# zachramsey/pm-rl

Hardware: AMD Instinct MI355X
Metric: env-steps/sec (whole node) at 65k envs x 30 assets; reward MAE vs CPU ref (higher is better)
Workload: dtype f64

## Files before the change

pm-rl_amd/csrc/step_relay.h:

```cpp
#pragma once
#include "env_step.h"
#include "scalar_vec.h"

namespace pmenv_dev {

struct RelayParams {
    uint32_t scal;
    uint32_t epoch;
    uint64_t* w;
    uint64_t* list;
    uint32_t* done;
    uint32_t spin;
    uint32_t rot;
    uint32_t grid;
    const int32_t* kp_in;
    int32_t* kp_out;
    const float* halo_in;
    float* halo_out;
    uint32_t* seq;
    int32_t* kp;
    float* halo;
    uint32_t B;
    uint32_t halo_stride;
    const float* obs;
    uint32_t par;
};
enum { kSeqD = 0, kSeqE = 1, kSeqV = 2, kSeqC = 3, kSeqEC = 4, kSeqHobs = 6 };

struct RelayCtx {
    uint32_t epoch;
    const int32_t* kp_in;
    int32_t* kp_out;
    const float* halo_in;
    float* halo_out;
};
template <bool SEQ>
__device__ __forceinline__ RelayCtx relay_ctx(const RelayParams& r) {
    RelayCtx c{r.epoch, r.kp_in, r.kp_out, r.halo_in, r.halo_out};
    if constexpr (SEQ) {
        const uint32_t par = __builtin_amdgcn_readfirstlane(r.seq[kSeqC]);
        c.epoch = __builtin_amdgcn_readfirstlane(r.seq[kSeqEC]);
        c.kp_in = r.kp + (size_t)par * r.B;
        c.kp_out = r.kp + (size_t)(par ^ 1u) * r.B;
        c.halo_in = r.halo + (size_t)par * r.halo_stride;
        c.halo_out = r.halo + (size_t)(par ^ 1u) * r.halo_stride;
    }
    return c;
}

struct KArgs {
    StepParams p;
    RelayParams r;
    uint32_t qtot;
};
__device__ __forceinline__ KArgs kargs() {
    typedef __attribute__((address_space(4))) const uint32_t KWord;
    KWord* ka = (KWord*)__builtin_amdgcn_kernarg_segment_ptr();
    asm volatile("" : "+s"(ka));
    uint32_t w[sizeof(KArgs) / 4];
#pragma unroll
    for (size_t i = 0; i < sizeof(KArgs) / 4; ++i) w[i] = ka[i];
    KArgs k;
    __builtin_memcpy(&k, w, sizeof(KArgs));
    return k;
}

constexpr uint32_t kStampSlots = 16, kStampMaxWg = 40960;
static __device__ uint64_t* g_relay_stamps;
template <bool ST, bool DRAIN = false>
__device__ __forceinline__ uint64_t relay_clock(uint32_t dep) {
    uint64_t t = 0;
    if constexpr (ST) {
        if constexpr (DRAIN)
            asm volatile("s_waitcnt vmcnt(0)\n\ts_memrealtime %0\n\ts_waitcnt lgkmcnt(0)" : "=s"(t) : "v"(dep) : "memory");
        else
            asm volatile("s_memrealtime %0\n\ts_waitcnt lgkmcnt(0)" : "=s"(t) : "v"(dep) : "memory");
    }
    return t;
}
template <bool ST, int K>
__device__ __forceinline__ void relay_stamps_put(uint32_t bid, uint32_t epoch, const uint64_t (&ts)[K]) {
    if constexpr (ST) {
        uint64_t* s = g_relay_stamps;
        if (s && threadIdx.x == 0 && bid < kStampMaxWg) {
#pragma unroll
            for (int k = 0; k < K; ++k) s[((size_t)(epoch % kStampSlots) * kStampMaxWg + bid) * 8 + k] = ts[k];
        }
    }
}

__device__ __forceinline__ void relay_put(uint64_t* w, uint32_t epoch, uint32_t bits) {
    __hip_atomic_store(w, ((uint64_t)epoch << 32) | bits, __ATOMIC_RELAXED, __HIP_MEMORY_SCOPE_AGENT);
}
__device__ __forceinline__ uint64_t relay_get(const uint64_t* w) {
    return __hip_atomic_load(const_cast<uint64_t*>(w), __ATOMIC_RELAXED, __HIP_MEMORY_SCOPE_AGENT);
}

__device__ __forceinline__ uint32_t relay_list_read(const RelayParams& r, uint32_t epoch) {
    __atomic_signal_fence(__ATOMIC_SEQ_CST);
    __builtin_amdgcn_s_waitcnt(0);
    __atomic_signal_fence(__ATOMIC_SEQ_CST);
    const uint64_t lw = relay_get(r.list);
    return (uint32_t)(lw >> 32) == epoch ? (uint32_t)lw : 0u;
}

template <int BLOCK, int KL, int KA, bool ST = false>
__device__ __forceinline__ uint32_t relay_scalar(const StepParams& p, const RelayParams& r, int s, uint32_t epoch,
                                                 int32_t* kp_out, uint64_t t_entry = 0) {
    uint64_t ts[3] = {t_entry, 0, 0};
    constexpr int EPW = 64 / KL, EPB = (BLOCK / 64) * EPW;
    const int lane = threadIdx.x & 63;
    const int b = s * EPB + (int)(threadIdx.x >> 6) * EPW + lane / KL;
    const int j = lane % KL;
    const int N = p.N;
    const bool env_ok = b < p.B;
    uint32_t listed;
    if constexpr (KA == 0) {
        const ScalarIn in = scalar_load<KL>(p, b, lane);
        const ScalarMid m = scalar_core<KL>(p, b, lane, in);
        if (env_ok && j < N) relay_put(r.w + (size_t)b * N + j, epoch, __float_as_uint(m.wp));
        if (env_ok && j == 0) kp_out[b] = m.k + 1;
        listed = relay_list_read(r, epoch);
        ts[1] = relay_clock<ST>(listed);
        scalar_tail<KL>(p, b, lane, in, m);
    } else {
        const VecIn<KA> in = vec_load<KL, KA, true>(p, b, lane);
        const VecMid<KA> m = vec_core<KL, KA, true>(p, b, lane, in);
#pragma unroll
        for (int e = 0; e < KA; ++e) {
            const int n = j + e * KL;
            if (env_ok && n < N) relay_put(r.w + (size_t)b * N + n, epoch, __float_as_uint(m.wp[e]));
        }
        if (env_ok && j == 0) kp_out[b] = in.k + 1;
        listed = relay_list_read(r, epoch);
        ts[1] = relay_clock<ST>(listed);
        vec_tail<KL, KA, true>(p, b, lane, in, m);
    }
    ts[2] = relay_clock<ST, true>(0);
    relay_stamps_put<ST>((uint32_t)s, epoch, ts);
    return listed;
}

template <int BLOCK, int V, int POL, bool OUT, bool ADOPT, bool ST = false>
__device__ __forceinline__ bool relay_tile(const StepParams& p, const RelayParams& r, uint32_t qtot, uint32_t spin, uint32_t t,
                                           uint32_t epoch, const int32_t* kp_in, const float* halo_in,
                                           float* halo_out, f4* sh4, f4* sh_bar, float* sh_wp, int32_t* sh_kc,
                                           int32_t* sh_ok, uint64_t t_entry = 0) {
    uint64_t ts[6] = {t_entry, 0, 0, 0, 0, 0};
    constexpr int kAux = POL == 1 ? 2 : 0;
    constexpr int CPW = BLOCK * V, F = 5;
    const int tid = threadIdx.x, lane = tid & 63, wave = tid >> 6;
    const uint32_t c0 = t * CPW;
    const uint32_t nblk = min((uint32_t)CPW, qtot - c0);
    const auto rs = make_rsrc(p.obs + (size_t)c0 * 4, nblk * 16u);
    f4 own[V];
#pragma unroll
    for (int v = 0; v < V; ++v) own[v] = buf_load4<kAux>(rs, (uint32_t)(64 * V * wave + 64 * v + lane) * 16u);
    const uint32_t ntiles = (qtot + CPW - 1) / CPW;
    const uint32_t nh = t + 1 < ntiles ? min(2u, qtot - c0 - nblk) : 0u;
    const float* hsrc = OUT ? p.obs + (size_t)(c0 + nblk) * 4 : halo_in + (size_t)t * 8;
    const f4 hal = buf_load4<0>(make_rsrc(hsrc, nh * 16u), tid < 2 ? (uint32_t)tid * 16u : 0xFFFFFFF0u);
    __builtin_amdgcn_sched_barrier(0);
    const int N = p.N, W = p.W, WF = W * F;
    const uint32_t per4 = (uint32_t)(N * WF) >> 2;
    const uint32_t b_lo = fdiv(c0, p.div_units);
    const uint32_t g_lo = b_lo * (uint32_t)N + fdiv(4u * (c0 - b_lo * per4), p.div_wf);
    const uint32_t ql = c0 + nblk - 1u;
    const uint32_t b_hi = fdiv(ql, p.div_units);
    const uint32_t g_hi = b_hi * (uint32_t)N + fdiv(4u * (ql - b_hi * per4) + 3u, p.div_wf);
    const bool mine = (uint32_t)tid <= g_hi - g_lo;
    const uint32_t g = g_lo + (mine ? (uint32_t)tid : 0u);
    const uint32_t b = g / (uint32_t)N, n = g - b * (uint32_t)N;
    const float* barb = env_bar(p, (int)b);
    const float nanv = __int_as_float(0x7fc00000);
    f4 xb = f4{nanv, nanv, nanv, nanv};
    int32_t kc = 0;
    uint64_t ww = 0;
    if (barb) xb = *reinterpret_cast<const f4*>(barb + (size_t)n * 4);
    kc = kp_in[b];
    ww = relay_get(r.w + g);
    bool ready = !mine || (uint32_t)(ww >> 32) == epoch;
    ts[1] = relay_clock<ST>((uint32_t)ww);
    for (uint32_t polls = 0; !ADOPT && !__all(ready) && polls < spin; ++polls) {
        __builtin_amdgcn_s_sleep(2);
        if (!ready) {
            ww = relay_get(r.w + g);
            ready = (uint32_t)(ww >> 32) == epoch;
        }
    }
    const bool wave_ok = __all(ready);
    ts[2] = relay_clock<ST>((uint32_t)ww);
    if (mine) {
        sh_bar[tid] = xb;
        sh_wp[tid] = __uint_as_float((uint32_t)ww);
        sh_kc[tid] = kc;
    }
#pragma unroll
    for (int v = 0; v < V; ++v) sh4[64 * V * wave + 64 * v + lane] = own[v];
    if (tid < 2) sh4[CPW + tid] = hal;
    if (lane == 0) sh_ok[wave] = wave_ok ? 1 : 0;
    __syncthreads();
    ts[3] = relay_clock<ST>(0);
    if constexpr (ADOPT) {
        bool tile_ok = true;
#pragma unroll
        for (int w = 0; w < BLOCK / 64; ++w) tile_ok = tile_ok && sh_ok[w] != 0;
        if (!tile_ok) return false;
        if (tid == 0)
            sh_ok[BLOCK / 64] = __hip_atomic_exchange(r.done + t, epoch, __ATOMIC_RELAXED, __HIP_MEMORY_SCOPE_AGENT) != epoch;
        __syncthreads();
        if (!sh_ok[BLOCK / 64]) return true;
    }
    const auto rd = OUT ? make_rsrc(p.obs_out + (size_t)c0 * 4, nblk * 16u) : rs;
    const bool first_out = !OUT && t > 0;
    bool ok = true;
#pragma unroll
    for (int v = 0; v < V; ++v) {
        const int j = 64 * V * wave + 64 * v + lane;
        const uint32_t q = min(c0 + (uint32_t)j, qtot - 1u);
        const uint32_t bq = fdiv(q, p.div_units);
        const uint32_t j0 = 4u * (q - bq * per4);
        const uint32_t row = fdiv(j0, p.div_wf);
        const int kk = (int)(j0 - row * (uint32_t)WF);
        const int i = (int)(bq * (uint32_t)N + row - g_lo);
        const f4 n1 = sh4[j + 1], n2 = sh4[j + 2];
        const float sh[4] = {n1.y, n1.z, n1.w, n2.x};
        const float un[4] = {own[v].x, own[v].y, own[v].z, own[v].w};
        f4 o = compose2(p, kk, sh_kc[i], un, sh, [&](f4& x, float& xwp) {
            x = sh_bar[i];
            xwp = sh_wp[i];
        });
        if (!ADOPT && v == 0) {
            int32_t okv = 1;
#pragma unroll
            for (int w = 0; w < BLOCK / 64; ++w) okv &= sh_ok[w];
            ok = __builtin_amdgcn_readfirstlane(okv) != 0;
        }
        buf_store4<kAux>(rd, ok ? (uint32_t)j * 16u : 0x80000000u, o);
        if (ok && first_out && j < 2) reinterpret_cast<f4*>(halo_out)[2 * (t - 1) + j] = o;
    }
    ts[4] = relay_clock<ST>(0);
    ts[5] = relay_clock<ST, true>(0);
    relay_stamps_put<ST>(r.scal + t, epoch, ts);
    return ok;
}

template <int BLOCK, int V, int POL, bool OUT, bool SEQ>
__device__ __forceinline__ void relay_adopt(f4* sh4, f4* sh_bar, float* sh_wp, int32_t* sh_kc, int32_t* sh_ok,
                                            uint32_t listed) {
    constexpr int kB = BLOCK / 64 + 1;
    const int wave = threadIdx.x >> 6;
    if ((threadIdx.x & 63) == 0) sh_ok[wave] = (int32_t)__builtin_amdgcn_readfirstlane(listed);
    __syncthreads();
    uint32_t n = 0;
#pragma unroll
    for (int w = 0; w < BLOCK / 64; ++w) n = max(n, (uint32_t)sh_ok[w]);
    if (n == 0) return;
    const KArgs ka = kargs();
    const RelayCtx c = relay_ctx<SEQ>(ka.r);
    for (uint32_t i = 0; i < n; ++i) {
        __syncthreads();
        if (threadIdx.x == 0) {
            const uint64_t e = relay_get(ka.r.list + 1 + i);
            int32_t t = (uint32_t)(e >> 32) == c.epoch ? (int32_t)(uint32_t)e : -1;
            if (t >= 0 && __hip_atomic_load(ka.r.done + t, __ATOMIC_RELAXED, __HIP_MEMORY_SCOPE_AGENT) == c.epoch)
                t = -1;
            sh_ok[kB] = t;
        }
        __syncthreads();
        const int32_t t = __builtin_amdgcn_readfirstlane(sh_ok[kB]);
        if (t >= 0)
            (void)relay_tile<BLOCK, V, POL, OUT, true>(ka.p, ka.r, ka.qtot, 0u, (uint32_t)t, c.epoch, c.kp_in, c.halo_in,
                                                       c.halo_out, sh4, sh_bar, sh_wp, sh_kc, sh_ok);
    }
}

template <int BLOCK, int V, int POL, bool OUT, bool SEQ>
__device__ __forceinline__ void relay_defer(uint32_t t, f4* sh4, f4* sh_bar, float* sh_wp, int32_t* sh_kc,
                                            int32_t* sh_ok) {
    const KArgs ka = kargs();
    const RelayCtx c = relay_ctx<SEQ>(ka.r);
    if (threadIdx.x == 0) {
        uint64_t lw = relay_get(ka.r.list), nw;
        do {
            nw = (uint32_t)(lw >> 32) == c.epoch ? lw + 1 : ((uint64_t)c.epoch << 32) | 1u;
        } while (!__hip_atomic_compare_exchange_strong(ka.r.list, &lw, nw, __ATOMIC_RELAXED, __ATOMIC_RELAXED,
                                                        __HIP_MEMORY_SCOPE_AGENT));
        const uint32_t slot = (uint32_t)(lw >> 32) == c.epoch ? (uint32_t)lw : 0u;
        relay_put(ka.r.list + 1 + slot, c.epoch, t);
        __atomic_signal_fence(__ATOMIC_SEQ_CST);
        __builtin_amdgcn_s_waitcnt(0);
        __atomic_signal_fence(__ATOMIC_SEQ_CST);
    }
    __syncthreads();
    (void)relay_tile<BLOCK, V, POL, OUT, true>(ka.p, ka.r, ka.qtot, 0u, t, c.epoch, c.kp_in, c.halo_in, c.halo_out, sh4,
                                               sh_bar, sh_wp, sh_kc, sh_ok);
}

template <int BLOCK, int V, int POL, bool OUT, int KL, int KA, int OCC = 1, bool SEQ = false, int ANY = 0>
__global__ __launch_bounds__(BLOCK) __attribute__((amdgpu_waves_per_eu(OCC))) void step_relay_kernel(
    StepParams p, RelayParams r, uint32_t qtot) {
    __shared__ f4 sh4[BLOCK * V + 2];
    __shared__ f4 sh_bar[BLOCK];
    __shared__ float sh_wp[BLOCK];
    __shared__ int32_t sh_kc[BLOCK];
    __shared__ int32_t sh_ok[BLOCK / 64 + 2];
    const RelayCtx c = relay_ctx<SEQ>(r);
    if constexpr (SEQ) {
        if (blockIdx.x == 0 && threadIdx.x == 0) {
            const uint64_t hobs = OUT ? 0ull : (uint64_t)(uintptr_t)r.obs;
            r.seq[kSeqD] = (uint32_t)((c.kp_in - r.kp) / r.B) ^ 1u;
            r.seq[kSeqE] = c.epoch;
            r.seq[kSeqV] = 1u;
            r.seq[kSeqHobs] = (uint32_t)hobs;
            r.seq[kSeqHobs + 1] = (uint32_t)(hobs >> 32);
        }
    }
    constexpr bool kSt = ANY == 2;
    const uint64_t t_entry = relay_clock<kSt>(0);
    uint32_t bid = blockIdx.x;
    if constexpr (ANY == 1) {
        bid += r.rot;
        if (bid >= r.grid) bid -= r.grid;
    }
    if (bid < r.scal) {
        const uint32_t listed = relay_scalar<BLOCK, KL, KA, kSt>(p, r, (int)bid, c.epoch, c.kp_out, t_entry);
        relay_adopt<BLOCK, V, POL, OUT, SEQ>(sh4, sh_bar, sh_wp, sh_kc, sh_ok, listed);
    } else if (!relay_tile<BLOCK, V, POL, OUT, false, kSt>(p, r, qtot, ANY == 1 ? r.spin : kRelaySpin, bid - r.scal, c.epoch,
                                                           c.kp_in, c.halo_in, c.halo_out, sh4, sh_bar, sh_wp, sh_kc,
                                                           sh_ok, t_entry)) {
        relay_defer<BLOCK, V, POL, OUT, SEQ>(bid - r.scal, sh4, sh_bar, sh_wp, sh_kc, sh_ok);
    }
}

static __global__ __launch_bounds__(256) void relay_prime_kernel(StepParams p, RelayParams r, int prime_kp, int seq) {
    uint32_t d = r.par;
    bool kp = prime_kp != 0, halo = p.halo != nullptr;
    if (seq) {
        d = __builtin_amdgcn_readfirstlane(r.seq[kSeqD]);
        const uint32_t e = __builtin_amdgcn_readfirstlane(r.seq[kSeqE]);
        const uint32_t v = __builtin_amdgcn_readfirstlane(r.seq[kSeqV]);
        const uint64_t hobs = (uint64_t)__builtin_amdgcn_readfirstlane(r.seq[kSeqHobs]) |
                              ((uint64_t)__builtin_amdgcn_readfirstlane(r.seq[kSeqHobs + 1]) << 32);
        kp = v == 0;
        halo = halo && (v == 0 || hobs != (uint64_t)(uintptr_t)p.obs);
        if (blockIdx.x == 0 && threadIdx.x == 0) {
            r.seq[kSeqC] = d;
            r.seq[kSeqEC] = e + 1u == 0u ? 1u : e + 1u;
        }
    }
    if (halo) {
        p.halo += (size_t)d * r.halo_stride;
        copy_halo(p);
    }
    if (kp) {
        int32_t* kpd = r.kp + (size_t)d * r.B;
        for (int b = blockIdx.x * blockDim.x + threadIdx.x; b < p.B; b += gridDim.x * blockDim.x) kpd[b] = p.k[b];
    }
}

}
```

Baseline: 105.0 million.

## Add uniform-shift fast path that scatters new row cells into LDS image

Adds a fast path to the non-adopt relay tile. When every row in the block agrees on whether the weight slot shifts, each row owner writes its new bar values and weight straight into the shared tile image. Every output vector is then just a four-float shifted read, with an optional keep-weight select, instead of the per-element compose2 with its fdiv index math and per-row lookups. The cost is an extra __syncthreads, more registers for the per-row cell offsets, and overwriting sh4, so the fallback path now reads own values back from shared memory.

```diff
diff --git a/pm-rl_amd/csrc/compose_cells.h b/pm-rl_amd/csrc/compose_cells.h
--- /dev/null
+++ b/pm-rl_amd/csrc/compose_cells.h
@@ -0,0 +1,57 @@
+#pragma once
+
+#include <stdint.h>
+
+#if defined(__HIPCC__)
+#define PMENV_CELLS_HD __host__ __device__ inline
+#else
+#define PMENV_CELLS_HD inline
+#endif
+
+namespace compose_cells {
+
+constexpr int kF = 5;
+constexpr int kCells = 5;
+constexpr int kNoWeight = 4;
+
+PMENV_CELLS_HD bool shape_ok(int64_t N, int64_t W) { return N >= 1 && W >= 2 && (N * W * kF) % 4 == 0; }
+
+PMENV_CELLS_HD bool shift_w(bool ring_storage, int32_t k, int W) { return !(ring_storage && k >= W - 1); }
+
+PMENV_CELLS_HD int32_t slot_pos(int32_t k, int W) { return (int32_t)(((uint32_t)k + 1u) % (uint32_t)W) * kF + (kF - 1); }
+
+struct RowCells {
+    int32_t off[kCells];
+    uint32_t in;
+    bool shift_w;
+};
+
+PMENV_CELLS_HD RowCells row_cells_rel(int W, int32_t img, int32_t rel, int32_t k, bool ring_storage) {
+    RowCells c;
+    const int32_t WF = W * kF;
+    c.shift_w = shift_w(ring_storage, k, W);
+    for (int f = 0; f < kF - 1; ++f) c.off[f] = rel + WF + f;
+    c.off[kF - 1] = c.shift_w ? rel + WF + (kF - 1) : rel + slot_pos(k, W);
+    c.in = 0;
+    for (int i = 0; i < kCells; ++i) c.in |= (uint32_t)(c.off[i] >= 0 && c.off[i] < img) << i;
+    return c;
+}
+
+PMENV_CELLS_HD RowCells row_cells(int64_t N, int W, uint64_t c0, int32_t img, uint64_t g, int32_t k, bool ring_storage) {
+    (void)N;
+    const int64_t WF = (int64_t)W * kF;
+    const int64_t rel = (int64_t)g * WF - 4 * (int64_t)c0;
+    if (rel <= -WF - kCells || rel >= (int64_t)img) {
+        RowCells c;
+        for (int i = 0; i < kCells; ++i) c.off[i] = -1;
+        c.in = 0;
+        c.shift_w = shift_w(ring_storage, k, W);
+        return c;
+    }
+    return row_cells_rel(W, img, (int32_t)rel, k, ring_storage);
+}
+
+PMENV_CELLS_HD int weight_elem(uint64_t q) { return (int)((q + 4u) % 5u); }
+PMENV_CELLS_HD int weight_elem_tile(uint32_t c0_mod5, uint32_t j) { return (int)((c0_mod5 + j + 4u) % 5u); }
+
+}
diff --git a/pm-rl_amd/csrc/step_relay.h b/pm-rl_amd/csrc/step_relay.h
--- a/pm-rl_amd/csrc/step_relay.h
+++ b/pm-rl_amd/csrc/step_relay.h
@@ -1,4 +1,7 @@
 #pragma once
+#include <type_traits>
+
+#include "compose_cells.h"
 #include "env_step.h"
 #include "scalar_vec.h"
 
@@ -164,7 +167,9 @@
     const int N = p.N, W = p.W, WF = W * F;
     const uint32_t per4 = (uint32_t)(N * WF) >> 2;
     const uint32_t b_lo = fdiv(c0, p.div_units);
-    const uint32_t g_lo = b_lo * (uint32_t)N + fdiv(4u * (c0 - b_lo * per4), p.div_wf);
+    const uint32_t f_lo = 4u * (c0 - b_lo * per4);
+    const uint32_t r_lo = fdiv(f_lo, p.div_wf);
+    const uint32_t g_lo = b_lo * (uint32_t)N + r_lo;
     const uint32_t ql = c0 + nblk - 1u;
     const uint32_t b_hi = fdiv(ql, p.div_units);
     const uint32_t g_hi = b_hi * (uint32_t)N + fdiv(4u * (ql - b_hi * per4) + 3u, p.div_wf);
@@ -189,6 +194,16 @@
         }
     }
     const bool wave_ok = __all(ready);
+    const bool ring_st = p.ring_mode == PMENV_RING_STORAGE;
+    const bool row_sh = compose_cells::shift_w(ring_st, kc, W);
+    int32_t vote = wave_ok ? 1 : 0;
+    compose_cells::RowCells rc{};
+    if constexpr (!ADOPT) {
+        vote |= (__all(!mine || row_sh) ? 2 : 0) | (__all(!mine || !row_sh) ? 4 : 0);
+        const int32_t rel = (int32_t)(r_lo * (uint32_t)WF) - (int32_t)f_lo + tid * WF;
+        rc = compose_cells::row_cells_rel(W, 4 * (CPW + 2), rel, kc, ring_st);
+        if (!mine) rc.in = 0;
+    }
     ts[2] = relay_clock<ST>((uint32_t)ww);
     if (mine) {
         sh_bar[tid] = xb;
@@ -198,7 +213,7 @@
 #pragma unroll
     for (int v = 0; v < V; ++v) sh4[64 * V * wave + 64 * v + lane] = own[v];
     if (tid < 2) sh4[CPW + tid] = hal;
-    if (lane == 0) sh_ok[wave] = wave_ok ? 1 : 0;
+    if (lane == 0) sh_ok[wave] = vote;
     __syncthreads();
     ts[3] = relay_clock<ST>(0);
     if constexpr (ADOPT) {
@@ -214,6 +229,49 @@
     const auto rd = OUT ? make_rsrc(p.obs_out + (size_t)c0 * 4, nblk * 16u) : rs;
     const bool first_out = !OUT && t > 0;
     bool ok = true;
+    if constexpr (!ADOPT) {
+        int32_t okv = 7;
+#pragma unroll
+        for (int w = 0; w < BLOCK / 64; ++w) okv &= sh_ok[w];
+        okv = __builtin_amdgcn_readfirstlane(okv);
+        ok = (okv & 1) != 0;
+        if (okv & 6) {
+            if (rc.in) {
+                float* img = reinterpret_cast<float*>(sh4);
+                const float pv[compose_cells::kCells] = {xb.x, xb.y, xb.z, xb.w, __uint_as_float((uint32_t)ww)};
+#pragma unroll
+                for (int i = 0; i < compose_cells::kCells; ++i)
+                    if (rc.in >> i & 1u) img[rc.off[i]] = pv[i];
+            }
+            __syncthreads();
+            const uint32_t c0m = c0 % 5u;
+            const uint32_t soff = ok ? 0u : 0x80000000u;
+            auto shift_all = [&](auto keep_w) {
+#pragma unroll
+                for (int v = 0; v < V; ++v) {
+                    const int j = 64 * V * wave + 64 * v + lane;
+                    const f4 n1 = sh4[j + 1], n2 = sh4[j + 2];
+                    f4 o = f4{n1.y, n1.z, n1.w, n2.x};
+                    if constexpr (decltype(keep_w)::value) {
+                        const f4 n0 = sh4[j];
+                        const int ew = compose_cells::weight_elem_tile(c0m, (uint32_t)j);
+                        o.x = pick(ew == 0, n0.x, o.x);
+                        o.y = pick(ew == 1, n0.y, o.y);
+                        o.z = pick(ew == 2, n0.z, o.z);
+                        o.w = pick(ew == 3, n0.w, o.w);
+                    }
+                    buf_store4<kAux>(rd, soff + (uint32_t)j * 16u, o);
+                    if (v == 0 && ok && first_out && j < 2) reinterpret_cast<f4*>(halo_out)[2 * (t - 1) + j] = o;
+                }
+            };
+            if (okv & 4) shift_all(std::true_type{});
+            else shift_all(std::false_type{});
+            ts[4] = relay_clock<ST>(0);
+            ts[5] = relay_clock<ST, true>(0);
+            relay_stamps_put<ST>(r.scal + t, epoch, ts);
+            return ok;
+        }
+    }
 #pragma unroll
     for (int v = 0; v < V; ++v) {
         const int j = 64 * V * wave + 64 * v + lane;
@@ -223,19 +281,14 @@
         const uint32_t row = fdiv(j0, p.div_wf);
         const int kk = (int)(j0 - row * (uint32_t)WF);
         const int i = (int)(bq * (uint32_t)N + row - g_lo);
+        const f4 n0 = ADOPT ? own[v] : sh4[j];
         const f4 n1 = sh4[j + 1], n2 = sh4[j + 2];
         const float sh[4] = {n1.y, n1.z, n1.w, n2.x};
-        const float un[4] = {own[v].x, own[v].y, own[v].z, own[v].w};
+        const float un[4] = {n0.x, n0.y, n0.z, n0.w};
         f4 o = compose2(p, kk, sh_kc[i], un, sh, [&](f4& x, float& xwp) {
             x = sh_bar[i];
             xwp = sh_wp[i];
         });
-        if (!ADOPT && v == 0) {
-            int32_t okv = 1;
-#pragma unroll
-            for (int w = 0; w < BLOCK / 64; ++w) okv &= sh_ok[w];
-            ok = __builtin_amdgcn_readfirstlane(okv) != 0;
-        }
         buf_store4<kAux>(rd, ok ? (uint32_t)j * 16u : 0x80000000u, o);
         if (ok && first_out && j < 2) reinterpret_cast<f4*>(halo_out)[2 * (t - 1) + j] = o;
     }
```

New measurement: 105.0 million (median of 2 runs). No clear change (+0.0%).
